# Li-Qingyun/RSCoTr

Hardware: AMD Instinct MI355X
Metric: images/sec MTL train step (Swin-T 512^2, bs=2/GPU) (higher is better)
Workload: dtype f32 (large products as three fp16 MFMAs on two-plane power-of-two-scaled splits of the fp32 operands, fp32 accumulate: fp32-FMA-class error; six bf16 MFMAs on three-plane splits where an operand has no range word)

## Files before the change

rscotr_amd/build.py:

```python
import hashlib
import os
import shutil
import subprocess
import sys

HERE = os.path.dirname(os.path.abspath(__file__))
CSRC = os.path.join(HERE, "csrc")
LIB = os.path.join(HERE, "librscotr.so")
STAMP = os.path.join(HERE, "librscotr.so.stamp")
ARCH = "gfx950"
FLAGS = ["-O3", "-std=c++17", "-fPIC", "-munsafe-fp-atomics", "-fno-fast-math",
         "-Wno-unused-result"]
HOST_FLAGS = ["-ffp-contract=off"]


def _sources():
    return sorted(os.path.join(CSRC, f) for f in os.listdir(CSRC)
                  if f.endswith(".hip") or f.endswith(".cpp"))


def _digest():
    h = hashlib.sha256()
    for p in _sources() + sorted(os.path.join(CSRC, f) for f in os.listdir(CSRC) if f.endswith(".h")) + \
            [os.path.join(HERE, "..", "include", "rscotr.h")]:
        h.update(p.encode())
        with open(p, "rb") as fh:
            h.update(fh.read())
    h.update(" ".join(FLAGS + HOST_FLAGS).encode())
    return h.hexdigest()


def find_hipcc():
    for cand in (os.environ.get("HIPCC"), shutil.which("hipcc"), "/opt/rocm/bin/hipcc"):
        if cand and os.path.exists(cand):
            return cand
    return None


def build_library(force=False, verbose=True):
    dig = _digest()
    if not force and os.path.exists(LIB) and os.path.exists(STAMP):
        with open(STAMP) as fh:
            if fh.read().strip() == dig:
                return LIB
    hipcc = find_hipcc()
    if hipcc is None:
        raise RuntimeError("hipcc not found: cannot build librscotr.so")
    objs = []
    objdir = os.path.join(HERE, "_obj")
    os.makedirs(objdir, exist_ok=True)
    procs = []
    hdr = hashlib.sha256()
    for h in sorted(os.path.join(CSRC, f) for f in os.listdir(CSRC) if f.endswith(".h")) + \
            [os.path.join(HERE, "..", "include", "rscotr.h")]:
        with open(h, "rb") as fh:
            hdr.update(fh.read())
    for src in _sources():
        obj = os.path.join(objdir, os.path.basename(src) + ".o")
        objs.append(obj)
        extra = HOST_FLAGS if src.endswith(".cpp") else []
        with open(src, "rb") as fh:
            odig = hashlib.sha256(fh.read() + hdr.digest() + " ".join(FLAGS + extra).encode()).hexdigest()
        ostamp = obj + ".stamp"
        if not force and os.path.exists(obj) and os.path.exists(ostamp) and open(ostamp).read().strip() == odig:
            continue
        with open(ostamp, "w") as fh:
            fh.write(odig)
        cmd = [hipcc, f"--offload-arch={ARCH}", *FLAGS, *extra, "-x", "hip", "-c", src, "-o", obj,
               "-I", CSRC, "-I", os.path.join(HERE, "..", "include")]
        if verbose:
            print("[rscotr build]", " ".join(cmd), flush=True)
        procs.append((src, subprocess.Popen(cmd, stdout=subprocess.PIPE, stderr=subprocess.STDOUT)))
    for src, p in procs:
        out, _ = p.communicate()
        if p.returncode != 0:
            os.remove(os.path.join(objdir, os.path.basename(src) + ".o.stamp"))
            raise RuntimeError(f"hipcc failed on {src}:\n{out.decode()}")
    cmd = [hipcc, f"--offload-arch={ARCH}", "-shared", "-fPIC", *objs, "-ldl", "-o", LIB]
    if verbose:
        print("[rscotr build]", " ".join(cmd), flush=True)
    subprocess.check_call(cmd)
    with open(STAMP, "w") as fh:
        fh.write(dig)
    return LIB


if __name__ == "__main__":
    build_library(force="--force" in sys.argv)
    print(LIB)
```

rscotr_amd/csrc/common.h:

```cpp
#pragma once
#include <hip/hip_runtime.h>
#include <stdint.h>
#include <stdio.h>
#include <stdarg.h>

#define RSCOTR_OK 0
#define RSCOTR_E_SHAPE (-1)
#define RSCOTR_E_ALIGN (-2)
#define RSCOTR_E_ARCH (-3)
#define RSCOTR_E_LAUNCH (-4)
#define RSCOTR_E_ARG (-5)

namespace rscotr {

char* err_buf();

inline int fail(int code, const char* fmt, ...) {
  va_list ap;
  va_start(ap, fmt);
  vsnprintf(err_buf(), 512, fmt, ap);
  va_end(ap);
  return code;
}

inline int check_launch(const char* what) {
  hipError_t e = hipGetLastError();
  if (e != hipSuccess) return fail(RSCOTR_E_LAUNCH, "%s: %s", what, hipGetErrorString(e));
  return RSCOTR_OK;
}

inline bool aligned16(const void* p) { return (reinterpret_cast<uintptr_t>(p) & 15u) == 0; }

constexpr int kWave = 64;

enum { PROF_GEMM = 0, PROF_MSDA_FWD = 1, PROF_MSDA_BWD = 2, PROF_HBM = 3, PROF_MFMA = 4, PROF_KINDS = 5 };
struct ProfScope {
  int slot;
  hipStream_t stream;
  ProfScope(int kind, double work, hipStream_t s, const char* fmt, ...);
  ~ProfScope();
};

template <int G>
__device__ __forceinline__ float group_sum(float v) {
#pragma unroll
  for (int o = G / 2; o > 0; o >>= 1) v += __shfl_xor(v, o, 64);
  return v;
}

template <int G>
__device__ __forceinline__ float group_max(float v) {
#pragma unroll
  for (int o = G / 2; o > 0; o >>= 1) v = fmaxf(v, __shfl_xor(v, o, 64));
  return v;
}

__device__ __forceinline__ float wave_sum(float v) { return group_sum<64>(v); }
__device__ __forceinline__ float wave_max(float v) { return group_max<64>(v); }

constexpr int kAmaxPlanes = 32;
constexpr int kAmaxStride = 16384;
constexpr int kRangeExpLo = 80;

__device__ __forceinline__ int range_byte(unsigned bits) {
  return min(max((int)((bits >> 23) & 0xffu), kRangeExpLo), kRangeExpLo + 4 * kAmaxPlanes - 1) - kRangeExpLo;
}
__device__ __forceinline__ void range_mark(unsigned* slot, int i) {
  reinterpret_cast<unsigned char*>(slot + (long)(i >> 2) * kAmaxStride)[i & 3] = 1;
}

__device__ __forceinline__ unsigned amax_fold(unsigned v) {
  int c = v ? 4 * (int)(threadIdx.x & (kAmaxPlanes - 1)) + ((31 - __clz((int)v)) >> 3) + 1 : 0;
#pragma unroll
  for (int o = kAmaxPlanes / 2; o > 0; o >>= 1) c = max(c, __shfl_xor(c, o, 64));
  c = __builtin_amdgcn_readfirstlane(c);
  return c ? (unsigned)(kRangeExpLo + c - 1) << 23 : 0u;
}
__device__ __forceinline__ unsigned amax_read(const unsigned* word) {
  return amax_fold(word[(long)(threadIdx.x & (kAmaxPlanes - 1)) * kAmaxStride]);
}
__device__ __forceinline__ float amax_hi(unsigned folded) { return folded ? __uint_as_float(folded + (1u << 23)) : 0.f; }

__device__ __forceinline__ void amax_commit(unsigned* slot, float amx) {
  if (!slot) return;
#pragma unroll
  for (int o = 32; o > 0; o >>= 1) amx = fmaxf(amx, __shfl_xor(amx, o, 64));
  if ((threadIdx.x & 63) == 0) {
    const unsigned b = __float_as_uint(amx) & 0x7fffffffu;
    if (b) range_mark(slot, range_byte(b));
  }
}

__device__ __forceinline__ float2 msda_location(const float* __restrict__ r, float2 o, const float* __restrict__ norm, int l, int P,
                                                int refdim) {
  float2 out;
  if (refdim == 2) {
    out.x = r[0] + o.x / norm[2 * l];
    out.y = r[1] + o.y / norm[2 * l + 1];
  } else {
    out.x = r[0] + o.x / (float)P * r[2] * 0.5f;
    out.y = r[1] + o.y / (float)P * r[3] * 0.5f;
  }
  return out;
}

__device__ __forceinline__ float amax4(float a, const float4& v) {
  return fmaxf(fmaxf(a, fmaxf(fabsf(v.x), fabsf(v.y))), fmaxf(fabsf(v.z), fabsf(v.w)));
}

}
```

rscotr_amd/csrc/gemm_h3.hip:

```cpp
#include "gemm_split_body.h"
#include "gemm_plan.h"

namespace rscotr {
template <int BM, int BN, bool AKM, bool BKM, int PIPE, bool EDGE = false, int OCC = 1, bool BPL = false>
__global__ __launch_bounds__(256, OCC) void gemm_h3_kernel(GemmParams p) {
  __shared__ __attribute__((aligned(16))) unsigned lds[bf16x6_lds_words<BM, BN, AKM, BKM, PIPE, true>()];
  gemm_bf16x6_body<BM, BN, AKM, BKM, PIPE, false, EDGE, true, BPL>(p, blockIdx.x, gridDim.x, lds);
}
template <bool AKM, bool BKM, bool EDGE = false>
__global__ __launch_bounds__(256) __attribute__((amdgpu_waves_per_eu(2, 2))) void gemm_h3_128_kernel(GemmParams p) {
  __shared__ __attribute__((aligned(16))) unsigned lds[bf16x6_lds_words<128, 128, AKM, BKM, 0, true>()];
  gemm_bf16x6_body<128, 128, AKM, BKM, 0, false, EDGE, true>(p, blockIdx.x, gridDim.x, lds);
}

void launch_h3(const GemmParams& p, const GemmPlan& pl, hipStream_t s) {
  if (pl.b_from_planes) {
    gemm_h3_kernel<64, 64, false, false, 2, false, 4, true><<<dim3(pl.nwg), 256, 0, s>>>(p);
    return;
  }
  with_split_cfg(pl, [&](auto bm, auto pipe, auto edge) {
    with_layout(pl.a_kmajor, pl.b_kmajor, [&](auto ak, auto bk) {
      constexpr int BM = decltype(bm)::value, PIPE = decltype(pipe)::value;
      constexpr bool EDGE = decltype(edge)::value, AK = decltype(ak)::value, BK = decltype(bk)::value;
      if constexpr (BM == 128) {
        gemm_h3_128_kernel<AK, BK, EDGE><<<dim3(pl.nwg), 256, 0, s>>>(p);
      } else if (PIPE == 2 && !EDGE && !AK) {
        gemm_h3_kernel<64, 64, false, BK, 2, false, 4><<<dim3(pl.nwg), 256, 0, s>>>(p);
      } else {
        gemm_h3_kernel<BM, BM, AK, BK, PIPE, EDGE><<<dim3(pl.nwg), 256, 0, s>>>(p);
      }
    });
  });
}
}
```

rscotr_amd/csrc/gemm_split_body.h:

```cpp
#pragma once
#include "gemm_common.h"
#include <type_traits>

namespace rscotr {
typedef __bf16 bf16x2_t __attribute__((ext_vector_type(2)));
template <int NPL>
__device__ __forceinline__ void split_pair(float a, float b, unsigned (&out)[3]) {
  const f32x2_t x = {a, b};
  const bf16x2_t h = __builtin_convertvector(x, bf16x2_t);
  out[0] = __builtin_bit_cast(unsigned, h);
  const f32x2_t r1 = x - __builtin_convertvector(h, f32x2_t);
  const bf16x2_t m = __builtin_convertvector(r1, bf16x2_t);
  out[1] = __builtin_bit_cast(unsigned, m);
  if (NPL == 3) {
    const f32x2_t r2 = r1 - __builtin_convertvector(m, f32x2_t);
    out[2] = __builtin_bit_cast(unsigned, __builtin_convertvector(r2, bf16x2_t));
  } else {
    out[2] = 0u;
  }
}

__device__ __forceinline__ unsigned cvt_pk_bf16(float lo, float hi) {
  const f32x2_t x = {lo, hi};
  return __builtin_bit_cast(unsigned, __builtin_convertvector(x, bf16x2_t));
}

template <int NPL>
__device__ __forceinline__ void split_rows4(const float4& e, const float4& o, uint4 (&out)[3]) {
  f32x2_t e01 = {e.x, e.y}, e23 = {e.z, e.w}, o01 = {o.x, o.y}, o23 = {o.z, o.w};
#pragma unroll
  for (int pl = 0; pl < NPL; ++pl) {
    const unsigned h0 = cvt_pk_bf16(e01.x, o01.x), h1 = cvt_pk_bf16(e01.y, o01.y);
    const unsigned h2 = cvt_pk_bf16(e23.x, o23.x), h3 = cvt_pk_bf16(e23.y, o23.y);
    out[pl] = make_uint4(h0, h1, h2, h3);
    if (pl + 1 < NPL) {
      const f32x2_t fe01 = {__uint_as_float(h0 << 16), __uint_as_float(h1 << 16)};
      const f32x2_t fe23 = {__uint_as_float(h2 << 16), __uint_as_float(h3 << 16)};
      const f32x2_t fo01 = {__uint_as_float(h0 & 0xffff0000u), __uint_as_float(h1 & 0xffff0000u)};
      const f32x2_t fo23 = {__uint_as_float(h2 & 0xffff0000u), __uint_as_float(h3 & 0xffff0000u)};
      e01 -= fe01; e23 -= fe23; o01 -= fo01; o23 -= fo23;
    }
  }
}

__device__ __forceinline__ void split_rows4_h(const float4& e, const float4& o, const H3Scale& k, uint4 (&out)[3]) {
  unsigned a[3], b[3], c[3], d[3];
  split_pair_h(e.x, o.x, k, a);
  split_pair_h(e.y, o.y, k, b);
  split_pair_h(e.z, o.z, k, c);
  split_pair_h(e.w, o.w, k, d);
  out[0] = make_uint4(a[0], b[0], c[0], d[0]);
  out[1] = make_uint4(a[1], b[1], c[1], d[1]);
}

template <int R, bool KM, int NPL, int SBK = 16, bool H16 = false>
struct SplitOperand {
  static_assert(!H16 || NPL == 2, "the fp16 split has two planes");
  static constexpr int LDR = SBK * NPL + 8;
  static constexpr int KP = SBK / 2;
  static constexpr int Q = SBK / 4;
  static constexpr int WORDS = KM ? NPL * KP * R : R * LDR / 2;
  static constexpr int ITEMS = KM ? KP * R / 4 : R * Q;
  static constexpr int NV = (ITEMS + 255) / 256;
  float4 v[NV], w[NV];

  template <bool EDGE = false>
  __device__ __forceinline__ void load(const float* __restrict__ P, int ld, int row0, int k0, int tid, int rlast = 0, int klim = 0) {
#pragma unroll
    for (int i = 0; i < NV; ++i) {
      const int idx = tid + i * 256;
      if (ITEMS % 256 == 0 || idx < ITEMS) {
        if (!KM) {
          const int row = EDGE ? min(row0 + idx / Q, rlast) : row0 + idx / Q;
          const int kk = k0 + (idx % Q) * 4;
          v[i] = *reinterpret_cast<const float4*>(P + (long)row * ld + (EDGE ? min(kk, klim - 4) : kk));
          if (EDGE && kk >= klim) v[i] = make_float4(0.f, 0.f, 0.f, 0.f);
        } else {
          const int kp = idx / (R / 4), r4 = (idx % (R / 4)) * 4;
          const int ka = k0 + 2 * kp, col = EDGE ? min(row0 + r4, rlast) : row0 + r4;
          if (!EDGE) {
            const float* src = P + (long)ka * ld + col;
            v[i] = *reinterpret_cast<const float4*>(src);
            w[i] = *reinterpret_cast<const float4*>(src + ld);
          } else {
            v[i] = *reinterpret_cast<const float4*>(P + (long)min(ka, klim - 1) * ld + col);
            w[i] = *reinterpret_cast<const float4*>(P + (long)min(ka + 1, klim - 1) * ld + col);
            if (ka >= klim) v[i] = make_float4(0.f, 0.f, 0.f, 0.f);
            if (ka + 1 >= klim) w[i] = make_float4(0.f, 0.f, 0.f, 0.f);
          }
        }
      }
    }
  }
  __device__ __forceinline__ void scale_k(const float* __restrict__ ks, int per, int k0, int tid, int klast = 0x7ffffffe) {
#pragma unroll
    for (int i = 0; i < NV; ++i) {
      const int idx = tid + i * 256;
      if (ITEMS % 256 == 0 || idx < ITEMS) {
        const int k = k0 + 2 * (idx / (R / 4));
        const float f0 = ks[min(k, klast) / per], f1 = ks[min(k + 1, klast) / per];
        v[i].x *= f0; v[i].y *= f0; v[i].z *= f0; v[i].w *= f0;
        w[i].x *= f1; w[i].y *= f1; w[i].z *= f1; w[i].w *= f1;
      }
    }
  }
  __device__ __forceinline__ void accum(float4& a, int tid, float f = 1.f) const {
    static_assert(!KM || 256 % (R / 4) == 0, "row sums assume one row group per thread");
#pragma unroll
    for (int i = 0; i < NV; ++i)
      if (ITEMS % 256 == 0 || tid + i * 256 < ITEMS) {
        a.x = fmaf(f, v[i].x + w[i].x, a.x); a.y = fmaf(f, v[i].y + w[i].y, a.y);
        a.z = fmaf(f, v[i].z + w[i].z, a.z); a.w = fmaf(f, v[i].w + w[i].w, a.w);
      }
  }
  __device__ __forceinline__ void store(unsigned* S, int tid, const H3Scale& hs = H3Scale{1.f, 2048.f}) const {
#pragma unroll
    for (int i = 0; i < NV; ++i) {
      const int idx = tid + i * 256;
      if (ITEMS % 256 == 0 || idx < ITEMS) {
        if (!KM) {
          const int row = idx / Q, kq = (idx % Q) * 4;
          unsigned ab[3], cd[3];
          if constexpr (H16) {
            split_pair_h(v[i].x, v[i].y, hs, ab);
            split_pair_h(v[i].z, v[i].w, hs, cd);
          } else {
            split_pair<NPL>(v[i].x, v[i].y, ab);
            split_pair<NPL>(v[i].z, v[i].w, cd);
          }
          unsigned* dst = S + (row * LDR + kq) / 2;
#pragma unroll
          for (int pl = 0; pl < NPL; ++pl) {
            uint2 q;
            q.x = ab[pl];
            q.y = cd[pl];
            *reinterpret_cast<uint2*>(dst + pl * (SBK / 2)) = q;
          }
        } else {
          const int kp = idx / (R / 4), r4 = (idx % (R / 4)) * 4;
          uint4 q[3];
          if constexpr (H16) split_rows4_h(v[i], w[i], hs, q);
          else split_rows4<NPL>(v[i], w[i], q);
#pragma unroll
          for (int pl = 0; pl < NPL; ++pl) *reinterpret_cast<uint4*>(S + (pl * KP + kp) * R + r4) = q[pl];
        }
      }
    }
  }
  static __device__ __forceinline__ void frag(const unsigned* S, int row, int g, int ks, bf16x8 (&f)[3]) {
    if (!KM) {
      const unsigned* q = S + (row * LDR + 16 * ks + 8 * g) / 2;
#pragma unroll
      for (int pl = 0; pl < NPL; ++pl) f[pl] = __builtin_bit_cast(bf16x8, *reinterpret_cast<const uint4*>(q + pl * (SBK / 2)));
    } else {
#pragma unroll
      for (int pl = 0; pl < NPL; ++pl) {
        const unsigned* q = S + (pl * KP + 8 * ks + 4 * g) * R + row;
        uint4 t;
        t.x = q[0]; t.y = q[R]; t.z = q[2 * R]; t.w = q[3 * R];
        f[pl] = __builtin_bit_cast(bf16x8, t);
      }
    }
  }
};

template <int R, int SBK>
struct PlaneOperandH {
  using Lay = SplitOperand<R, false, 2, SBK, true>;
  static_assert(R == 64 && SBK == 32, "one 32-byte piece per thread");
  static constexpr int WORDS = Lay::WORDS, KP = Lay::KP;
  typedef float vec4 __attribute__((ext_vector_type(4)));
  vec4 v0, v1;
  template <bool EDGE = false>
  __device__ __forceinline__ void load(const float* __restrict__ P, int ld, int row0, int k0, int tid, int = 0, int = 0) {
    const vec4* src = reinterpret_cast<const vec4*>(P) + ((long)(k0 / SBK) * ld + row0) * 8 + tid * 2;
    v0 = src[0];
    v1 = src[1];
  }
  __device__ __forceinline__ void store(unsigned* S, int tid, const H3Scale& = H3Scale{1.f, 2048.f}) const {
    vec4* dst = reinterpret_cast<vec4*>(S + (tid >> 2) * (Lay::LDR / 2) + (tid & 3) * 8);
    dst[0] = v0;
    dst[1] = v1;
  }
  static __device__ __forceinline__ void frag(const unsigned* S, int row, int g, int ks, bf16x8 (&f)[3]) { Lay::frag(S, row, g, ks, f); }
};

__device__ const float bf16x6_one = 1.f;
template <int PIPE> constexpr int bf16x6_bk() { return PIPE == 2 ? 32 : PIPE == 0 ? X6_BK0 : 16; }
constexpr int X6_D2 = 2, H3_VPM = 8, H3_DPM = 2;
template <int PIPE> constexpr int bf16x6_depth() { return PIPE == 2 ? X6_D2 : 1; }

template <int BM, int BN, bool AKM, bool BKM, int PIPE, bool H16 = false>
constexpr int bf16x6_lds_words() {
  constexpr int NPL = H16 ? 2 : 3;
  return (PIPE ? 2 : 1) * (SplitOperand<BM, AKM, NPL, bf16x6_bk<PIPE>(), H16>::WORDS + SplitOperand<BN, BKM, NPL, bf16x6_bk<PIPE>(), H16>::WORDS);
}

template <int BM, int BN, bool AKM, bool BKM, int PIPE, bool SLAB, bool EDGE = false, bool H16 = false, bool BPL = false>
__device__ __forceinline__ void gemm_bf16x6_body(GemmParams& p, const int bx, const int gx, unsigned* lds) {
  constexpr int NPL = H16 ? 2 : 3, SBK = bf16x6_bk<PIPE>(), D = bf16x6_depth<PIPE>();
  constexpr int MT = BM / 64, NT = BN / 64;
  using OA = SplitOperand<BM, AKM, NPL, SBK, H16>;
  static_assert(!BPL || (H16 && !BKM && !EDGE && PIPE == 2), "B from planes: the interior pipelined fp16 kernel");
  using OB = typename std::conditional<BPL, PlaneOperandH<BN, SBK>, SplitOperand<BN, BKM, NPL, SBK, H16>>::type;
  H3Scale ha{1.f, 2048.f}, hb{1.f, 2048.f};
  float inva = 1.f, invb = 1.f;
  unsigned ra = 0u, rb = 0u;
  if constexpr (H16) {
    ra = p.amax_a[(long)(threadIdx.x & (kAmaxPlanes - 1)) * kAmaxStride];
    rb = p.amax_b[(long)(threadIdx.x & (kAmaxPlanes - 1)) * kAmaxStride];
  }
  auto h3_scales = [&]() {
    if constexpr (H16) {
      const int ea = h3_scale_exp(amax_fold(ra)), eb = h3_scale_exp(amax_fold(rb));
      ha.sc = __uint_as_float((unsigned)ea << 23); ha.sc2 = __uint_as_float((unsigned)(ea + 11) << 23);
      hb.sc = __uint_as_float((unsigned)eb << 23); hb.sc2 = __uint_as_float((unsigned)(eb + 11) << 23);
      inva = __uint_as_float((unsigned)(254 - ea) << 23); invb = __uint_as_float((unsigned)(254 - eb) << 23);
    }
  };
  constexpr int NBUF = PIPE ? 2 : 1;
  unsigned* sA[2] = {lds, lds + (NBUF - 1) * OA::WORDS};
  unsigned* sB[2] = {lds + NBUF * OA::WORDS, lds + NBUF * OA::WORDS + (NBUF - 1) * OB::WORDS};
  const int tid = threadIdx.x, lane = tid & 63, wave = tid >> 6;
  const int wm = wave >> 1, wn = wave & 1;
  const int tiles_n = EDGE ? (p.N + BN - 1) / BN : p.N / BN;
  const int alast = EDGE ? (AKM ? p.M - 4 : p.M - 1) : 0, blast = EDGE ? (BKM ? p.N - 4 : p.N - 1) : 0;
  int tile, split = 0;
  if (p.splits == 1) {
    tile = xcd_swizzle(bx, gx);
  } else {
    const int x = bx & 7, j = bx >> 3;
    const int q = p.tiles >> 3, r = p.tiles & 7, run = q + (r ? 1 : 0);
    const int nt = q + (x < r ? 1 : 0);
    split = j / run;
    const int tl = j - split * run;
    if (tl >= nt) return;
    tile = (x < r ? x * (q + 1) : r * (q + 1) + (x - r) * q) + tl;
  }
  const int m0 = (tile / tiles_n) * BM, n0 = (tile % tiles_n) * BN;
  const int kbeg = split * p.ksplit_len;
  const int kend = min(p.K, kbeg + p.ksplit_len);
  const int nk = EDGE ? (kend - kbeg + SBK - 1) / SBK : (kend - kbeg) / SBK;
  const int klast = EDGE ? p.K - 1 : 0x7ffffffe;

  f32x16 acc[MT][NT];
  f32x16 acc2[H16 ? MT : 1][H16 ? NT : 1];
#pragma unroll
  for (int i = 0; i < MT; ++i)
#pragma unroll
    for (int j = 0; j < NT; ++j)
#pragma unroll
      for (int r = 0; r < 16; ++r) {
        acc[i][j][r] = 0.f;
        if constexpr (H16) acc2[i][j][r] = 0.f;
      }
  OA las[D];
  OB lbs[D];
  OA& la = las[0];
  OB& lb = lbs[0];
  const bool do_rs = AKM && p.rowsum && n0 == 0;
  float4 rs = make_float4(0.f, 0.f, 0.f, 0.f);
  const int fr = lane & 31, g = lane >> 5;
  auto fetch = [&](int t) {
    la.template load<EDGE>(p.A, p.lda, m0, kbeg + t * SBK, tid, alast, p.K);
    lb.template load<EDGE>(p.B, p.ldb, n0, kbeg + t * SBK, tid, blast, p.K);
    if (AKM && p.kscale) la.scale_k(p.kscale, p.krows_per, kbeg + t * SBK, tid, klast);
  };
  auto stage = [&](unsigned* a_s, unsigned* b_s) {
    if (AKM && do_rs) la.accum(rs, tid);
    la.store(a_s, tid, ha);
    lb.store(b_s, tid, hb);
  };
  auto mma = [&](const unsigned* a_s, const unsigned* b_s) {
#pragma unroll
    for (int ks = 0; ks < SBK / 16; ++ks) {
      bf16x8 af[MT][3], bf[NT][3];
#pragma unroll
      for (int i = 0; i < MT; ++i) OA::frag(a_s, wm * (BM / 2) + i * 32 + fr, g, ks, af[i]);
#pragma unroll
      for (int j = 0; j < NT; ++j) OB::frag(b_s, wn * (BN / 2) + j * 32 + fr, g, ks, bf[j]);
      if constexpr (H16) {
#pragma unroll
        for (int tm = 0; tm < 3; ++tm)
#pragma unroll
          for (int i = 0; i < MT; ++i)
#pragma unroll
            for (int j = 0; j < NT; ++j) {
              const f16x8 a = __builtin_bit_cast(f16x8, af[i][tm == 0 ? 1 : 0]), b = __builtin_bit_cast(f16x8, bf[j][tm == 1 ? 1 : 0]);
              if (tm < 2) acc2[i][j] = __builtin_amdgcn_mfma_f32_32x32x16_f16(a, b, acc2[i][j], 0, 0, 0);
              else acc[i][j] = __builtin_amdgcn_mfma_f32_32x32x16_f16(a, b, acc[i][j], 0, 0, 0);
            }
        continue;
      }
      constexpr int PA[6] = {2, 0, 1, 1, 0, 0}, PB[6] = {0, 2, 1, 0, 1, 0};
#pragma unroll
      for (int tm = 0; tm < 6; ++tm)
#pragma unroll
        for (int i = 0; i < MT; ++i)
#pragma unroll
          for (int j = 0; j < NT; ++j)
            acc[i][j] = __builtin_amdgcn_mfma_f32_32x32x16_bf16(af[i][PA[tm]], bf[j][PB[tm]], acc[i][j], 0, 0, 0);
    }
  };
  if (PIPE == 2) {
    constexpr int U = (D % 2 == 0) ? D : 2 * D;
    constexpr int NMFMA = MT * NT * (H16 ? 3 : 6) * (SBK / 16);
    constexpr int VPM = H16 ? H3_VPM : 4, DPM = H16 ? H3_DPM : 1;
    const float* ksp = (AKM && p.kscale) ? p.kscale : &bf16x6_one;
    const int ksper = (AKM && p.kscale) ? p.krows_per : 0x7fffffff;
#pragma unroll
    for (int d = 0; d < D; ++d) {
      const int tt = min(d, nk - 1);
      las[d].template load<EDGE>(p.A, p.lda, m0, kbeg + tt * SBK, tid, alast, p.K);
      lbs[d].template load<EDGE>(p.B, p.ldb, n0, kbeg + tt * SBK, tid, blast, p.K);
    }
    h3_scales();
    if (AKM) las[0].scale_k(ksp, ksper, kbeg, tid, klast);
    if (AKM) las[0].accum(rs, tid);
    las[0].store(sA[0], tid, ha);
    lbs[0].store(sB[0], tid, hb);
    __syncthreads();
    for (int t0 = 0; t0 < nk; t0 += U) {
#pragma unroll
      for (int s = 0; s < U; ++s) {
        const int t = t0 + s;
        if (t < nk) {
          {
            const int tt = min(t + D, nk - 1);
            las[s % D].template load<EDGE>(p.A, p.lda, m0, kbeg + tt * SBK, tid, alast, p.K);
            lbs[s % D].template load<EDGE>(p.B, p.ldb, n0, kbeg + tt * SBK, tid, blast, p.K);
          }
          mma(sA[s & 1], sB[s & 1]);
          if (AKM) las[(s + 1) % D].scale_k(ksp, ksper, kbeg + min(t + 1, nk - 1) * SBK, tid, klast);
          if (AKM) las[(s + 1) % D].accum(rs, tid, t + 1 < nk ? 1.f : 0.f);
          las[(s + 1) % D].store(sA[(s + 1) & 1], tid, ha);
          lbs[(s + 1) % D].store(sB[(s + 1) & 1], tid, hb);
#pragma unroll
          for (int i = 0; i < NMFMA; ++i) {
            __builtin_amdgcn_sched_group_barrier(0x008, 1, 0);
            __builtin_amdgcn_sched_group_barrier(0x002, VPM, 0);
            __builtin_amdgcn_sched_group_barrier(0x200, DPM, 0);
          }
          __syncthreads();
        }
      }
    }
  } else if (PIPE) {
    fetch(0);
    h3_scales();
    stage(sA[0], sB[0]);
    if (nk > 1) fetch(1);
    __syncthreads();
    for (int t = 0; t < nk; ++t) {
      const bool odd = t & 1;
      mma(odd ? sA[1] : sA[0], odd ? sB[1] : sB[0]);
      if (t + 1 < nk) {
        stage(odd ? sA[0] : sA[1], odd ? sB[0] : sB[1]);
        if (t + 2 < nk) fetch(t + 2);
      }
      __syncthreads();
    }
  } else {
    fetch(0);
    h3_scales();
    for (int t = 0; t < nk; ++t) {
      __syncthreads();
      stage(sA[0], sB[0]);
      if (t + 1 < nk) fetch(t + 1);
      __syncthreads();
      mma(sA[0], sB[0]);
    }
  }

  if (AKM && do_rs) {
    __syncthreads();
    constexpr int KL = 256 / (BM / 4) < OA::KP ? 256 / (BM / 4) : OA::KP;
    float4* red = reinterpret_cast<float4*>(lds);
    if (tid < KL * BM / 4) red[tid] = rs;
    __syncthreads();
    if (tid < BM) {
      const float* rf = reinterpret_cast<const float*>(lds);
      float v = 0.f;
#pragma unroll
      for (int k = 0; k < KL; ++k) v += rf[k * BM + tid];
      const int m = m0 + tid;
      if (!EDGE || m < p.M) {
        if (p.splits > 1 || SLAB) p.rs_slabs[(long)split * p.M + m] = v;
        else p.rowsum[m] = p.rowsum_acc ? p.rowsum[m] + v : v;
      }
    }
  }

  if constexpr (H16) {
#pragma unroll
    for (int i = 0; i < MT; ++i)
#pragma unroll
      for (int j = 0; j < NT; ++j)
#pragma unroll
        for (int r = 0; r < 16; ++r) acc[i][j][r] = fmaf(acc2[i][j][r], 0x1p-11f, acc[i][j][r]) * inva * invb;
  }
  if (p.splits > 1 || SLAB) {
    float* slab = p.slabs + (long)split * p.M * p.N;
#pragma unroll
    for (int i = 0; i < MT; ++i)
#pragma unroll
      for (int j = 0; j < NT; ++j) {
        const int n = n0 + wn * (BN / 2) + j * 32 + fr;
#pragma unroll
        for (int r = 0; r < 16; ++r) {
          const int m = m0 + wm * (BM / 2) + i * 32 + (r & 3) + 8 * (r >> 2) + 4 * g;
          if (!EDGE || (m < p.M && n < p.N)) slab[(long)m * p.N + n] = acc[i][j][r];
        }
      }
    return;
  }
  if constexpr (BM == 128 && BN == 128 && !EDGE) {
    if (p.act == ACT_RELU_BITS || p.act == ACT_RELU_GRAD_BITS) {
      const bool fwd = p.act == ACT_RELU_BITS;
      const long widx = ((long)(m0 / 128) * (p.N / 128) + n0 / 128) * 256 + tid;
      unsigned long long bits = fwd ? 0ull : reinterpret_cast<const unsigned long long*>(p.aux)[widx];
      float amx = 0.f;
#pragma unroll
      for (int i = 0; i < MT; ++i)
#pragma unroll
        for (int j = 0; j < NT; ++j) {
          const int n = n0 + wn * (BN / 2) + j * 32 + fr;
          const float bv = p.bias ? p.bias[n] : 0.f;
          float* crow = p.C + (long)(m0 + wm * (BM / 2) + i * 32 + 4 * g) * p.ldc + n;
#pragma unroll
          for (int r = 0; r < 16; ++r) {
            const int b = (i * NT + j) * 16 + r;
            float v = acc[i][j][r] + bv;
            if (fwd) {
              v = fmaxf(v, 0.f);
              bits |= (unsigned long long)(v > 0.f) << b;
            } else {
              v = ((bits >> b) & 1ull) ? v : 0.f;
            }
            crow[(long)((r & 3) + 8 * (r >> 2)) * p.ldc] = v;
            amx = fmaxf(amx, fabsf(v));
          }
        }
      if (fwd) reinterpret_cast<unsigned long long*>(p.pre)[widx] = bits;
      amax_commit(p.amax_out, amx);
      return;
    }
  }
  const bool plain = !p.pre && p.act == ACT_NONE && !p.resid && !p.accumulate && !p.rowscale && !p.C2;
  const bool one_extra = BM == 64 && !p.C2 &&
                         ((p.act == ACT_RELU_GRAD || p.act == ACT_GELU_GRAD) ? 1 : 0) + (p.resid ? 1 : 0) + (p.accumulate ? 1 : 0) == 1;
  const bool noload = !plain && (p.act == ACT_NONE || p.act == ACT_RELU || p.act == ACT_GELU) && !p.resid && !p.accumulate &&
                      !p.rowscale && !p.C2;
  float amx = 0.f;
#pragma unroll
  for (int i = 0; i < MT; ++i)
#pragma unroll
    for (int j = 0; j < NT; ++j) {
      const int n = n0 + wn * (BN / 2) + j * 32 + fr;
      if (EDGE && n >= p.N) continue;
      const float bv = p.bias ? p.bias[n] : 0.f;
      const int mb = m0 + wm * (BM / 2) + i * 32 + 4 * g;
      float* crow = p.C + (long)mb * p.ldc + n;
      if (one_extra) {
        epilogue_tile16<EDGE>(p, acc[i][j], bv, mb, n, amx);
        __builtin_amdgcn_sched_barrier(0);
      } else if (noload) {
        epilogue_noload16<EDGE>(p, acc[i][j], bv, mb, n, amx);
      } else if (plain) {
#pragma unroll
        for (int r = 0; r < 16; ++r)
          if (!EDGE || mb + (r & 3) + 8 * (r >> 2) < p.M) {
            const float v = acc[i][j][r] + bv;
            crow[(long)((r & 3) + 8 * (r >> 2)) * p.ldc] = v;
            amx = fmaxf(amx, fabsf(v));
          }
      } else {
#pragma unroll
        for (int g4 = 0; g4 < 4; ++g4) {
          float v[4];
#pragma unroll
          for (int u = 0; u < 4; ++u) v[u] = acc[i][j][4 * g4 + u] + bv;
          epilogue_rows4<EDGE>(p, v, mb + 8 * g4, n, amx);
          __builtin_amdgcn_sched_barrier(0);
        }
      }
    }
  amax_commit(p.amax_out, amx);
}
}
```

rscotr_amd/ops/deferred.py:

```python
import ctypes
from typing import NamedTuple

import numpy as np
import torch

from .._lib import _TRACE
from .core import ACT_NONE, _ptr, _stream, lib
from .ranges import RANGES
from .state import STATE


class Slab(NamedTuple):
    slab: int
    rs_slab: int
    out: int
    rowsum: int
    M: int
    N: int
    ldc: int
    splits: int


class LnPart(NamedTuple):
    part: int
    dw: int
    db: int
    rows: int
    C: int


class WattnPart(NamedTuple):
    part: int
    dtable: int
    dbias: int
    heads: int
    C: int
    rows: int


class GroupProblem(NamedTuple):
    a: int
    b: int
    out: int
    rowsum: int
    kscale: int
    M: int
    N: int
    K: int
    lda: int
    ldb: int
    krows_per: int
    range_a: int = 0
    range_b: int = 0


class _DeferredCombine:

    BLOCK = 256 << 20
    MAX_TABLES = 64
    GROUP_MAX_OUT = 160000
    GROUP_MAX_OUT_SHORT = 2500000
    GROUP_SHORT_K = 4096
    GROUP_EDGE = 48
    GROUP_TARGET_WGS = 4608

    def __init__(self):
        self.enabled = True
        self.blocks, self.cur, self.off = [], 0, 0
        self.entries, self.notify, self.cache = [], [], {}
        self.ln_entries, self.ln_cache = [], {}
        self.pin = False
        self.pinned = set()
        self.group_enabled = True
        self.group_x6 = 1
        self.group, self.group_keep, self.group_cache = [], [], {}
        self.group_amax, self.amax_cache = {}, {}
        self.pinned_pool, self.pinned_live = [], []
        self.captured = []
        self.wattn_entries, self.wattn_cache = [], {}

    def grouped_size(self, M, N, K):
        return M * N <= self.GROUP_MAX_OUT or (K <= self.GROUP_SHORT_K and M * N <= self.GROUP_MAX_OUT_SHORT)

    def split_member(self, M, N, K):
        return bool(self.group_x6 and K >= 512 and K % 16 == 0 and M % 4 == 0 and N % 4 == 0 and min(M, N) >= self.GROUP_EDGE)

    def _plan_group(self):
        probs = [GroupProblem(*p) for p in self.group]

        def kind(p):
            if not (self.split_member(p.M, p.N, p.K) and p.lda % 4 == 0 and p.ldb % 4 == 0 and p.a % 16 == 0 and p.b % 16 == 0):
                return 0
            return 7 if p.range_a and p.range_b and RANGES.enabled else 6

        def row(m, first):
            if m is None:
                return [0] * 12 + [first, 0, 0, 0]
            p = m['p']
            return [p.a, p.b, m['slab'], m['rs_slab'], p.kscale, p.M, p.N, p.K, p.lda, p.ldb, m['klen'], m['splits'], first,
                    max(p.krows_per, 1), m['ranges'], m['wgs']]

        kinds = [kind(p) for p in probs]
        tiles = [((p.M + 127) // 128) * ((p.N + 127) // 128) if k else ((p.M + 63) // 64) * ((p.N + 63) // 64)
                 for k, p in zip(kinds, probs)]
        dev = self.group_keep[0].device
        launches, ents = [], []
        for variant in (0, 6, 7):
            big = 4 if variant else 1
            klen_t = max(256, -(-sum(t * p.K * big for t, k, p in zip(tiles, kinds, probs) if k == variant) // self.GROUP_TARGET_WGS))
            kq = 32 if variant else 16
            members = []
            for t, k, p in zip(tiles, kinds, probs):
                if k != variant:
                    continue
                sp = max(1, -(-p.K // max(256, klen_t // big)))
                klen = -(-(-(-p.K // sp)) // kq) * kq
                sp = -(-p.K // klen)
                if sp == 1:
                    klen = p.K
                slab = self.reserve(sp * (p.M * p.N + p.M) * 4, dev)
                rs_slab = slab + sp * p.M * p.N * 4 if p.rowsum else 0
                rng = ((RANGES.index(p.range_a) + 1) << 32 | (RANGES.index(p.range_b) + 1)) if variant == 7 else 0
                members.append(dict(p=p, slab=slab, rs_slab=rs_slab, klen=klen, splits=sp, ranges=rng, wgs=t * sp))
                ents.append(Slab(slab, rs_slab, p.out, p.rowsum, p.M, p.N, p.N, sp))
            if members:
                members.sort(key=lambda m: -m['wgs'])
                members += [None] * (-len(members) % 8)
                rows, first = [], 0
                for b0 in range(0, len(members), 8):
                    rows += [row(m, first) for m in members[b0:b0 + 8]]
                    first += 8 * members[b0]['wgs']
                flops = float(sum(2.0 * m['p'].M * m['p'].N * m['p'].K for m in members if m is not None))
                launches.append((self._upload(np.asarray(rows, dtype=np.int64), dev), len(rows), first, variant, flops))
        return launches, ents

    def prepare_capture(self, n=4):
        while len(self.pinned_pool) < n:
            self.pinned_pool.append(torch.empty((4096, 16), dtype=torch.int64).pin_memory())

    @staticmethod
    def _copy(arr, dev):
        return torch.from_numpy(arr).to(dev)

    def _upload(self, arr, dev):
        if dev.type == 'cuda' and torch.cuda.is_current_stream_capturing():
            assert arr.size <= 4096 * 16, f'a table of {arr.size} words does not fit a staging buffer'
            assert self.pinned_pool, ('no staging buffer left for a table built during a capture: the pool is exhausted '
                                      f'({len(self.pinned_live)} taken), or DEFER.prepare_capture() did not run')
            host = self.pinned_pool.pop()
            stage = host.view(-1)[:arr.size].view(arr.shape)
            stage.copy_(torch.from_numpy(arr))
            d = torch.empty(arr.shape, dtype=torch.int64, device=dev)
            d.copy_(stage, non_blocking=True)
            self.pinned_live.append(host)
            return d
        return self._copy(arr, dev)

    def forget_captured(self):
        for cache, sig in self.captured:
            cache.pop(sig, None)
            self.pinned.discard(sig)
        self.captured = []

    def keep_captured(self):
        self.captured = []

    def _remember(self, cache, sig, hit):
        if sig not in cache and torch.cuda.is_available() and torch.cuda.is_current_stream_capturing():
            self.captured.append((cache, sig))
        if self.pin:
            self.pinned.add(sig)
        if sig not in cache:
            cache[sig] = hit
            if len(cache) > self.MAX_TABLES:
                for k in list(cache):
                    if len(cache) <= self.MAX_TABLES:
                        break
                    if k not in self.pinned and k != sig:
                        del cache[k]

    def reserve(self, nbytes, device):
        nbytes = (nbytes + 255) // 256 * 256
        while True:
            if self.cur == len(self.blocks):
                self.blocks.append(torch.empty(max(self.BLOCK, nbytes) // 4, dtype=torch.float32, device=device))
            b = self.blocks[self.cur]
            if self.off + nbytes <= b.numel() * 4:
                ptr = b.data_ptr() + self.off
                self.off += nbytes
                return ptr
            self.cur, self.off = self.cur + 1, 0

    def pending(self):
        return bool(self.entries or self.ln_entries or self.group or self.wattn_entries)

    def drop(self):
        self.entries, self.notify, self.ln_entries = [], [], []
        self.group, self.group_keep = [], []
        self.group_amax = {}
        self.wattn_entries = []
        self.cur = self.off = 0

    @staticmethod
    def _rounds(entries, dests):
        seen, rounds = {}, []
        for e in entries:
            ds = [d for d in dests(e) if d]
            k = max([seen.get(d, 0) for d in ds] or [0])
            for d in ds:
                seen[d] = k + 1
            while len(rounds) <= k:
                rounds.append([])
            rounds[k].append(e)
        return rounds

    def _flush_queue(self, entries, cache, kind, dests, plan, entry_point, upload):
        sig = tuple(entries)
        hit = cache.get(sig)
        if hit is None:
            dev = self.blocks[0].device
            hit = []
            for ents in self._rounds([kind(*e) for e in entries], dests):
                arrays, scalars = plan(ents)
                hit.append((tuple(upload(a, dev) for a in arrays), scalars))
        self._remember(cache, sig, hit)
        for tabs, scalars in hit:
            lib.call(entry_point, *(t.data_ptr() for t in tabs), *scalars, _stream())

    @staticmethod
    def _workgroups(ents, count):
        return np.asarray([(r, c) for r, e in enumerate(ents) for c in range(count(e))], dtype=np.int32)

    def _plan_ln(self, ents):
        wg = self._workgroups(ents, lambda e: (2 * e.C + 63) // 64)
        return (np.asarray(ents, dtype=np.int64), wg), (len(wg),)

    def _plan_wattn(self, ents):
        rows, first = [], 0
        for e in ents:
            rows.append(tuple(e) + (first,) + (0,) * 9)
            first += e.heads
        return (np.asarray(rows, dtype=np.int64),), (len(rows), first)

    def _plan_splitk(self, ents):
        wg = self._workgroups(ents, lambda e: (max(e.M * e.N // 4, e.M) + 255) // 256)
        nbytes = float(sum((e.splits + 2) * (e.M * e.N + e.M) * 4 for e in ents))
        return (np.asarray(ents, dtype=np.int64), wg), (len(wg), nbytes)

    def group_range(self, t, rows, cols, ld):
        s = RANGES.slot_of(t)
        if s:
            return s
        sink = STATE.grad_sink
        if sink is not None and sink.is_param_ptr(t.data_ptr()):
            return RANGES.of(t, rows, cols, ld)
        key = (t.data_ptr(), rows, cols, ld)
        s = self.group_amax.get(key)
        if s is None:
            s = self.group_amax[key] = RANGES.new_slot(t.device)
            if _TRACE:
                import sys
                end = t.storage_offset() * 4 + ((rows - 1) * ld + cols) * 4
                print(f'[group_range] {tuple(t.shape)} rows={rows} cols={cols} ld={ld} last byte {end} of storage {t.untyped_storage().nbytes()}'
                      + ('  <-- OUT OF BOUNDS' if end > t.untyped_storage().nbytes() else ''), file=sys.stderr, flush=True)
        return s

    def _measure_group(self):
        sig = tuple(self.group_amax.items())
        hit = self.amax_cache.get(sig)
        if hit is None:
            rows_, first = [], 0
            for (ptr, rows, cols, ld), slot in self.group_amax.items():
                rows_.append((ptr, rows, cols, ld, slot, first))
                first += max(1, min(128, rows * cols // 65536))
            hit = (self._upload(np.asarray(rows_, dtype=np.int64), self.group_keep[0].device), len(rows_), first)
        self._remember(self.amax_cache, sig, hit)
        table, n, total = hit
        lib.call('rscotr_amax_group', table.data_ptr(), n, total, _stream())
        RANGES.stats['grouped'] = RANGES.stats.get('grouped', 0) + n
        self.group_amax = {}

    def _flush_group(self):
        if self.group_amax:
            self._measure_group()
        sig = (tuple(self.group), self.cur, self.off)
        hit = self.group_cache.get(sig)
        if hit is None:
            hit = self._plan_group() + (self.cur, self.off)
        launches, ents, self.cur, self.off = hit
        self._remember(self.group_cache, sig, hit)
        for table, n, total, variant, flops in launches:
            lib.call('rscotr_gemm_dw_group', table.data_ptr(), n, total, variant, flops, RANGES.base if variant == 7 else 0,
                     _stream())
        self.entries.extend(ents)
        self.group, self.group_keep = [], []

    def flush(self):
        if self.group:
            self._flush_group()
        if self.ln_entries:
            self._flush_queue(self.ln_entries, self.ln_cache, LnPart, lambda e: (e.dw, e.db), self._plan_ln,
                              'rscotr_layernorm_flush', self._copy)
            self.ln_entries = []
        if self.wattn_entries:
            self._flush_queue(self.wattn_entries, self.wattn_cache, WattnPart, lambda e: (e.dtable, e.dbias), self._plan_wattn,
                              'rscotr_swin_wattn_flush', self._upload)
            self.wattn_entries = []
        if self.entries:
            self._flush_queue(self.entries, self.cache, Slab, lambda e: (e.out, e.rowsum), self._plan_splitk,
                              'rscotr_splitk_flush', self._copy)
        notify, self.notify = self.notify, []
        self.entries = []
        self.cur = self.off = 0
        if STATE.grad_sink is not None:
            for i in notify:
                STATE.grad_sink._on_ready(i)


DEFER = _DeferredCombine()


def _ranges_invalidated():
    DEFER.group = [GroupProblem(*p)._replace(range_a=0, range_b=0) for p in DEFER.group]
    DEFER.group_amax = {}


RANGES.on_invalidate.append(_ranges_invalidated)


def flush_deferred():
    if DEFER.pending() or DEFER.notify:
        DEFER.flush()


def _in_arena(t):
    sink = STATE.grad_sink
    if sink is None or t is None:
        return False
    lo = sink.flat_g.data_ptr()
    return lo <= t.data_ptr() < lo + sink.flat_g.numel() * 4


def _try_defer_dw(A, B, out, M, N, K, lda, ldb, rowsum, kscale, krows_per, nws):
    if not DEFER.enabled or STATE.side is not None or N % 4 or out.data_ptr() % 16 or not _in_arena(out):
        return False
    if DEFER.group_enabled and DEFER.grouped_size(M, N, K) and K >= 16:
        sa = sb = 0
        if DEFER.split_member(M, N, K) and RANGES.enabled:
            sa, sb = DEFER.group_range(A, K, M, lda), DEFER.group_range(B, K, N, ldb)
            lo_r, hi_r = RANGES.base, RANGES.base + 4 * RANGES.STRIDE
            if not (lo_r <= sa < hi_r and lo_r <= sb < hi_r):
                sa = sb = 0
        DEFER.group.append(GroupProblem(A.data_ptr(), B.data_ptr(), out.data_ptr(), _ptr(rowsum), _ptr(kscale), M, N, K, lda, ldb,
                                        int(krows_per), sa, sb))
        DEFER.group_keep.extend(t for t in (A, B, kscale) if t is not None)
        return True
    if nws == 0:
        return False
    ptr = DEFER.reserve(nws, A.device)
    splits = ctypes.c_int32(1)
    sa = sb = 0
    if RANGES.wanted(M, N, K, lda, ldb, 1, 1, ACT_NONE, False, False, kscale is not None, nws):
        sa, sb = RANGES.of(A, K, M, lda), RANGES.of(B, K, N, ldb)
    lib.call('rscotr_gemm_f32_dw_slabs_r', A.data_ptr(), B.data_ptr(), out.data_ptr(), M, N, K, lda, ldb, N, _ptr(rowsum),
             _ptr(kscale), int(krows_per), ptr, nws, ctypes.byref(splits), sa, sb, _stream())
    sp = splits.value
    if sp > 1:
        DEFER.entries.append(Slab(ptr, ptr + sp * M * N * 4 if rowsum is not None else 0, out.data_ptr(), _ptr(rowsum), M, N, N, sp))
    return True
```

Before: 210.6.

## Double-buffer register fetch sets in 128x128 fp16 split GEMM with buffer loads

For the 128x128 K-major fp16 three-MFMA GEMM kernel, the main loop now keeps two register sets of global loads in flight. The next tile's loads are issued while the current one is staged and multiplied. Loads use raw buffer loads with precomputed per-thread offsets and hardware bounds clamping, and k-scale factors are fetched ahead through the constant address space. Opaque asm barriers pin registers so the compiler does not spill. The build now checks resource-usage remarks and fails if these kernels use scratch. A fallback single-set variant handles leading dimensions of 2^26 or more, which overflow the 32-bit offsets, and the grouped planner avoids the range kind in that case. The cost is higher register pressure, at two waves per EU.

```diff
diff --git a/rscotr_amd/build.py b/rscotr_amd/build.py
--- a/rscotr_amd/build.py
+++ b/rscotr_amd/build.py
@@ -12,6 +12,18 @@
 FLAGS = ["-O3", "-std=c++17", "-fPIC", "-munsafe-fp-atomics", "-fno-fast-math",
          "-Wno-unused-result"]
 HOST_FLAGS = ["-ffp-contract=off"]
+REMARK_FLAGS = ["-Rpass-analysis=kernel-resource-usage"]
+NO_SCRATCH = {"gemm_h3.hip": ("gemm_h3_128_kernel",), "gemm_group.hip": ("gemm_h3_group_kernel",)}
+
+
+def scratch_report(remarks, names):
+    out, cur = {}, None
+    for line in remarks.splitlines():
+        if "Function Name:" in line:
+            cur = line.split("Function Name:")[1].split()[0]
+        elif "ScratchSize [bytes/lane]:" in line and cur is not None and any(n in cur for n in names):
+            out[cur] = int(line.split("ScratchSize [bytes/lane]:")[1].split()[0])
+    return out
 
 
 def _sources():
@@ -58,7 +70,7 @@
     for src in _sources():
         obj = os.path.join(objdir, os.path.basename(src) + ".o")
         objs.append(obj)
-        extra = HOST_FLAGS if src.endswith(".cpp") else []
+        extra = HOST_FLAGS if src.endswith(".cpp") else REMARK_FLAGS if os.path.basename(src) in NO_SCRATCH else []
         with open(src, "rb") as fh:
             odig = hashlib.sha256(fh.read() + hdr.digest() + " ".join(FLAGS + extra).encode()).hexdigest()
         ostamp = obj + ".stamp"
@@ -76,6 +88,14 @@
         if p.returncode != 0:
             os.remove(os.path.join(objdir, os.path.basename(src) + ".o.stamp"))
             raise RuntimeError(f"hipcc failed on {src}:\n{out.decode()}")
+        names = NO_SCRATCH.get(os.path.basename(src))
+        if names:
+            report = scratch_report(out.decode(), names)
+            spilled = {k: v for k, v in report.items() if v}
+            if not report or spilled:
+                os.remove(os.path.join(objdir, os.path.basename(src) + ".o.stamp"))
+                raise RuntimeError(f"{src}: kernels that must not use scratch do (bytes per lane: {spilled}), or no resource-usage "
+                                   f"remark was found for {names}: see h3_two_tiles in csrc/gemm_split_body.h")
     cmd = [hipcc, f"--offload-arch={ARCH}", "-shared", "-fPIC", *objs, "-ldl", "-o", LIB]
     if verbose:
         print("[rscotr build]", " ".join(cmd), flush=True)
diff --git a/rscotr_amd/csrc/common.h b/rscotr_amd/csrc/common.h
--- a/rscotr_amd/csrc/common.h
+++ b/rscotr_amd/csrc/common.h
@@ -69,12 +69,19 @@
   reinterpret_cast<unsigned char*>(slot + (long)(i >> 2) * kAmaxStride)[i & 3] = 1;
 }
 
+__device__ __forceinline__ int amax_fold_code(unsigned v, int sub) { return v ? 4 * sub + ((31 - __clz((int)v)) >> 3) + 1 : 0; }
+__device__ __forceinline__ unsigned amax_fold_bits(int c) { return c ? (unsigned)(kRangeExpLo + c - 1) << 23 : 0u; }
 __device__ __forceinline__ unsigned amax_fold(unsigned v) {
-  int c = v ? 4 * (int)(threadIdx.x & (kAmaxPlanes - 1)) + ((31 - __clz((int)v)) >> 3) + 1 : 0;
+  int c = amax_fold_code(v, (int)(threadIdx.x & (kAmaxPlanes - 1)));
 #pragma unroll
   for (int o = kAmaxPlanes / 2; o > 0; o >>= 1) c = max(c, __shfl_xor(c, o, 64));
-  c = __builtin_amdgcn_readfirstlane(c);
-  return c ? (unsigned)(kRangeExpLo + c - 1) << 23 : 0u;
+  return amax_fold_bits(__builtin_amdgcn_readfirstlane(c));
+}
+__device__ __forceinline__ unsigned amax_fold_lane(unsigned v, int lane) {
+  int c = amax_fold_code(v, lane & (kAmaxPlanes - 1));
+#pragma unroll
+  for (int o = kAmaxPlanes / 2; o > 0; o >>= 1) c = max(c, __builtin_amdgcn_ds_bpermute((lane ^ o) << 2, c));
+  return amax_fold_bits(__builtin_amdgcn_readfirstlane(c));
 }
 __device__ __forceinline__ unsigned amax_read(const unsigned* word) {
   return amax_fold(word[(long)(threadIdx.x & (kAmaxPlanes - 1)) * kAmaxStride]);
diff --git a/rscotr_amd/csrc/gemm_h3.hip b/rscotr_amd/csrc/gemm_h3.hip
--- a/rscotr_amd/csrc/gemm_h3.hip
+++ b/rscotr_amd/csrc/gemm_h3.hip
@@ -7,10 +7,10 @@
   __shared__ __attribute__((aligned(16))) unsigned lds[bf16x6_lds_words<BM, BN, AKM, BKM, PIPE, true>()];
   gemm_bf16x6_body<BM, BN, AKM, BKM, PIPE, false, EDGE, true, BPL>(p, blockIdx.x, gridDim.x, lds);
 }
-template <bool AKM, bool BKM, bool EDGE = false>
+template <bool AKM, bool BKM, bool EDGE = false, bool ONESET = false>
 __global__ __launch_bounds__(256) __attribute__((amdgpu_waves_per_eu(2, 2))) void gemm_h3_128_kernel(GemmParams p) {
   __shared__ __attribute__((aligned(16))) unsigned lds[bf16x6_lds_words<128, 128, AKM, BKM, 0, true>()];
-  gemm_bf16x6_body<128, 128, AKM, BKM, 0, false, EDGE, true>(p, blockIdx.x, gridDim.x, lds);
+  gemm_bf16x6_body<128, 128, AKM, BKM, 0, false, EDGE, true, false, ONESET>(p, blockIdx.x, gridDim.x, lds);
 }
 
 void launch_h3(const GemmParams& p, const GemmPlan& pl, hipStream_t s) {
@@ -23,7 +23,8 @@
       constexpr int BM = decltype(bm)::value, PIPE = decltype(pipe)::value;
       constexpr bool EDGE = decltype(edge)::value, AK = decltype(ak)::value, BK = decltype(bk)::value;
       if constexpr (BM == 128) {
-        gemm_h3_128_kernel<AK, BK, EDGE><<<dim3(pl.nwg), 256, 0, s>>>(p);
+        if (AK && BK && (p.lda >= (1 << 26) || p.ldb >= (1 << 26))) gemm_h3_128_kernel<AK, BK, EDGE, AK && BK><<<dim3(pl.nwg), 256, 0, s>>>(p);
+        else gemm_h3_128_kernel<AK, BK, EDGE><<<dim3(pl.nwg), 256, 0, s>>>(p);
       } else if (PIPE == 2 && !EDGE && !AK) {
         gemm_h3_kernel<64, 64, false, BK, 2, false, 4><<<dim3(pl.nwg), 256, 0, s>>>(p);
       } else {
diff --git a/rscotr_amd/csrc/gemm_split_body.h b/rscotr_amd/csrc/gemm_split_body.h
--- a/rscotr_amd/csrc/gemm_split_body.h
+++ b/rscotr_amd/csrc/gemm_split_body.h
@@ -92,6 +92,27 @@
       }
     }
   }
+  __device__ __forceinline__ unsigned thread_offset(int ld, int row0, int tid, bool edge, int rlast) const {
+    static_assert(!KM || ITEMS % 256 == 0, "whole items per thread");
+    const int col = row0 + (tid % (R / 4)) * 4;
+    return 4u * (unsigned)(2 * (tid / (R / 4)) * ld + (edge ? min(col, rlast) : col));
+  }
+  static __device__ __forceinline__ float4 load_row(const float* P, int ld, int krow, int klim, unsigned off) {
+    typedef unsigned vec4u __attribute__((ext_vector_type(4)));
+    const long left = 4l * ld * max(klim - krow, 0);
+    const __amdgpu_buffer_rsrc_t d = __builtin_amdgcn_make_buffer_rsrc(const_cast<float*>(P + (long)krow * ld), 0,
+                                                                        (int)(unsigned)min(left, 0xffffffffl), 0x00020000);
+    const vec4u t = __builtin_amdgcn_raw_buffer_load_b128(d, (int)off, 0, 0);
+    return make_float4(__uint_as_float(t.x), __uint_as_float(t.y), __uint_as_float(t.z), __uint_as_float(t.w));
+  }
+  __device__ __forceinline__ void load_rows(const float* __restrict__ P, int ld, int k0, int klim, unsigned off) {
+#pragma unroll
+    for (int i = 0; i < NV; ++i) {
+      const int krow = k0 + i * (2 * 256 / (R / 4));
+      v[i] = load_row(P, ld, krow, klim, off);
+      w[i] = load_row(P, ld, krow + 1, klim, off);
+    }
+  }
   __device__ __forceinline__ void scale_k(const float* __restrict__ ks, int per, int k0, int tid, int klast = 0x7ffffffe) {
 #pragma unroll
     for (int i = 0; i < NV; ++i) {
@@ -102,6 +123,32 @@
         v[i].x *= f0; v[i].y *= f0; v[i].z *= f0; v[i].w *= f0;
         w[i].x *= f1; w[i].y *= f1; w[i].z *= f1; w[i].w *= f1;
       }
+    }
+  }
+  __device__ __forceinline__ void scale_k_fetch(const float* __restrict__ ks, int per, int k0, int wave, int klast, float (&f)[4 * NV]) const {
+    static_assert(!KM || R == 128, "two k pairs per wavefront");
+#pragma unroll
+    for (int i = 0; i < NV; ++i) {
+      const int kb = k0 + 4 * wave + i * (2 * 256 / (R / 4));
+      int k = min(kb, klast), q = k / per, r = k - q * per;
+#pragma unroll
+      for (int j = 0; j < 4; ++j) {
+        const int kn = min(kb + j, klast);
+        if (kn != k) {
+          k = kn;
+          if (++r == per) { r = 0; ++q; }
+        }
+        f[4 * i + j] = *(const __attribute__((address_space(4))) float*)(ks + q);
+      }
+    }
+  }
+  __device__ __forceinline__ void scale_k_apply(const float (&f)[4 * NV], int tid) {
+    const bool hi = (tid / (R / 4)) & 1;
+#pragma unroll
+    for (int i = 0; i < NV; ++i) {
+      const float f0 = hi ? f[4 * i + 2] : f[4 * i], f1 = hi ? f[4 * i + 3] : f[4 * i + 1];
+      v[i].x *= f0; v[i].y *= f0; v[i].z *= f0; v[i].w *= f0;
+      w[i].x *= f1; w[i].y *= f1; w[i].z *= f1; w[i].w *= f1;
     }
   }
   __device__ __forceinline__ void accum(float4& a, int tid, float f = 1.f) const {
@@ -189,6 +236,8 @@
 template <int PIPE> constexpr int bf16x6_bk() { return PIPE == 2 ? 32 : PIPE == 0 ? X6_BK0 : 16; }
 constexpr int X6_D2 = 2, H3_VPM = 8, H3_DPM = 2;
 template <int PIPE> constexpr int bf16x6_depth() { return PIPE == 2 ? X6_D2 : 1; }
+template <int BM, int BN, bool AKM, bool BKM, int PIPE, bool EDGE, bool H16>
+constexpr bool h3_two_tiles() { return H16 && PIPE == 0 && BM == 128 && BN == 128 && AKM && BKM; }
 
 template <int BM, int BN, bool AKM, bool BKM, int PIPE, bool H16 = false>
 constexpr int bf16x6_lds_words() {
@@ -196,9 +245,10 @@
   return (PIPE ? 2 : 1) * (SplitOperand<BM, AKM, NPL, bf16x6_bk<PIPE>(), H16>::WORDS + SplitOperand<BN, BKM, NPL, bf16x6_bk<PIPE>(), H16>::WORDS);
 }
 
-template <int BM, int BN, bool AKM, bool BKM, int PIPE, bool SLAB, bool EDGE = false, bool H16 = false, bool BPL = false>
+template <int BM, int BN, bool AKM, bool BKM, int PIPE, bool SLAB, bool EDGE = false, bool H16 = false, bool BPL = false, bool ONESET = false>
 __device__ __forceinline__ void gemm_bf16x6_body(GemmParams& p, const int bx, const int gx, unsigned* lds) {
-  constexpr int NPL = H16 ? 2 : 3, SBK = bf16x6_bk<PIPE>(), D = bf16x6_depth<PIPE>();
+  constexpr bool TWO = !ONESET && h3_two_tiles<BM, BN, AKM, BKM, PIPE, EDGE, H16>();
+  constexpr int NPL = H16 ? 2 : 3, SBK = bf16x6_bk<PIPE>(), D = TWO ? 2 : bf16x6_depth<PIPE>();
   constexpr int MT = BM / 64, NT = BN / 64;
   using OA = SplitOperand<BM, AKM, NPL, SBK, H16>;
   static_assert(!BPL || (H16 && !BKM && !EDGE && PIPE == 2), "B from planes: the interior pipelined fp16 kernel");
@@ -212,7 +262,14 @@
   }
   auto h3_scales = [&]() {
     if constexpr (H16) {
-      const int ea = h3_scale_exp(amax_fold(ra)), eb = h3_scale_exp(amax_fold(rb));
+      if constexpr (TWO) {
+        int ln = (int)__lane_id();
+        asm volatile("" : "+v"(ln));
+        ra = amax_fold_lane(ra, ln); rb = amax_fold_lane(rb, ln);
+      } else {
+        ra = amax_fold(ra); rb = amax_fold(rb);
+      }
+      const int ea = h3_scale_exp(ra), eb = h3_scale_exp(rb);
       ha.sc = __uint_as_float((unsigned)ea << 23); ha.sc2 = __uint_as_float((unsigned)(ea + 11) << 23);
       hb.sc = __uint_as_float((unsigned)eb << 23); hb.sc2 = __uint_as_float((unsigned)(eb + 11) << 23);
       inva = __uint_as_float((unsigned)(254 - ea) << 23); invb = __uint_as_float((unsigned)(254 - eb) << 23);
@@ -221,8 +278,8 @@
   constexpr int NBUF = PIPE ? 2 : 1;
   unsigned* sA[2] = {lds, lds + (NBUF - 1) * OA::WORDS};
   unsigned* sB[2] = {lds + NBUF * OA::WORDS, lds + NBUF * OA::WORDS + (NBUF - 1) * OB::WORDS};
-  const int tid = threadIdx.x, lane = tid & 63, wave = tid >> 6;
-  const int wm = wave >> 1, wn = wave & 1;
+  int tid = threadIdx.x, lane = tid & 63, wave = tid >> 6;
+  int wm = wave >> 1, wn = wave & 1;
   const int tiles_n = EDGE ? (p.N + BN - 1) / BN : p.N / BN;
   const int alast = EDGE ? (AKM ? p.M - 4 : p.M - 1) : 0, blast = EDGE ? (BKM ? p.N - 4 : p.N - 1) : 0;
   int tile, split = 0;
@@ -260,7 +317,7 @@
   OB& lb = lbs[0];
   const bool do_rs = AKM && p.rowsum && n0 == 0;
   float4 rs = make_float4(0.f, 0.f, 0.f, 0.f);
-  const int fr = lane & 31, g = lane >> 5;
+  int fr = lane & 31, g = lane >> 5;
   auto fetch = [&](int t) {
     la.template load<EDGE>(p.A, p.lda, m0, kbeg + t * SBK, tid, alast, p.K);
     lb.template load<EDGE>(p.B, p.ldb, n0, kbeg + t * SBK, tid, blast, p.K);
@@ -272,13 +329,15 @@
     lb.store(b_s, tid, hb);
   };
   auto mma = [&](const unsigned* a_s, const unsigned* b_s) {
+    int ra0 = wm * (BM / 2) + fr, rb0 = wn * (BN / 2) + fr;
+    if constexpr (TWO) asm volatile("" : "+v"(ra0), "+v"(rb0));
 #pragma unroll
     for (int ks = 0; ks < SBK / 16; ++ks) {
       bf16x8 af[MT][3], bf[NT][3];
 #pragma unroll
-      for (int i = 0; i < MT; ++i) OA::frag(a_s, wm * (BM / 2) + i * 32 + fr, g, ks, af[i]);
-#pragma unroll
-      for (int j = 0; j < NT; ++j) OB::frag(b_s, wn * (BN / 2) + j * 32 + fr, g, ks, bf[j]);
+      for (int i = 0; i < MT; ++i) OA::frag(a_s, ra0 + i * 32, g, ks, af[i]);
+#pragma unroll
+      for (int j = 0; j < NT; ++j) OB::frag(b_s, rb0 + j * 32, g, ks, bf[j]);
       if constexpr (H16) {
 #pragma unroll
         for (int tm = 0; tm < 3; ++tm)
@@ -360,6 +419,56 @@
       }
       __syncthreads();
     }
+  } else if constexpr (TWO) {
+    float kf[4 * OA::NV];
+    const unsigned offa = la.thread_offset(p.lda, m0, tid, EDGE, alast);
+    const unsigned offb = lb.thread_offset(p.ldb, n0, tid, EDGE, blast);
+    const int wave_u = __builtin_amdgcn_readfirstlane(tid >> 6);
+    auto factors = [&](int t) {
+      if (p.kscale) la.scale_k_fetch(p.kscale, p.krows_per, kbeg + t * SBK, wave_u, klast, kf);
+    };
+    auto fetch2 = [&](auto set, int t) {
+      constexpr int S = decltype(set)::value;
+      const int k0 = __builtin_amdgcn_readfirstlane(kbeg + t * SBK);
+      las[S].load_rows(p.A, p.lda, k0, kend, offa);
+      lbs[S].load_rows(p.B, p.ldb, k0, kend, offb);
+    };
+    auto stage2 = [&](auto set) {
+      constexpr int S = decltype(set)::value;
+#pragma unroll
+      for (int i = 0; i < OA::NV; ++i) {
+        asm volatile("" : "+v"(las[S].v[i].x), "+v"(las[S].v[i].y), "+v"(las[S].v[i].z), "+v"(las[S].v[i].w));
+        asm volatile("" : "+v"(las[S].w[i].x), "+v"(las[S].w[i].y), "+v"(las[S].w[i].z), "+v"(las[S].w[i].w));
+        asm volatile("" : "+v"(lbs[S].v[i].x), "+v"(lbs[S].v[i].y), "+v"(lbs[S].v[i].z), "+v"(lbs[S].v[i].w));
+        asm volatile("" : "+v"(lbs[S].w[i].x), "+v"(lbs[S].w[i].y), "+v"(lbs[S].w[i].z), "+v"(lbs[S].w[i].w));
+      }
+      if (p.kscale) las[S].scale_k_apply(kf, tid);
+      if (do_rs) las[S].accum(rs, tid);
+      las[S].store(sA[0], tid, ha);
+      lbs[S].store(sB[0], tid, hb);
+    };
+    constexpr std::integral_constant<int, 0> s0{};
+    constexpr std::integral_constant<int, 1> s1{};
+    factors(0);
+    fetch2(s0, 0);
+    fetch2(s1, 1);
+    h3_scales();
+    for (int t = 0; t < nk; t += 2) {
+      __syncthreads();
+      stage2(s0);
+      if (t + 1 < nk) factors(t + 1);
+      fetch2(s0, t + 2);
+      __syncthreads();
+      mma(sA[0], sB[0]);
+      if (t + 1 < nk) {
+        __syncthreads();
+        stage2(s1);
+        if (t + 2 < nk) factors(t + 2);
+        fetch2(s1, t + 3);
+        __syncthreads();
+        mma(sA[0], sB[0]);
+      }
+    }
   } else {
     fetch(0);
     h3_scales();
@@ -372,6 +481,10 @@
     }
   }
 
+  if constexpr (TWO) {
+    asm volatile("" : "+v"(tid));
+    lane = tid & 63; wave = tid >> 6; wm = wave >> 1; wn = wave & 1; fr = lane & 31; g = lane >> 5;
+  }
   if (AKM && do_rs) {
     __syncthreads();
     constexpr int KL = 256 / (BM / 4) < OA::KP ? 256 / (BM / 4) : OA::KP;
diff --git a/rscotr_amd/ops/deferred.py b/rscotr_amd/ops/deferred.py
--- a/rscotr_amd/ops/deferred.py
+++ b/rscotr_amd/ops/deferred.py
@@ -91,7 +91,7 @@
         def kind(p):
             if not (self.split_member(p.M, p.N, p.K) and p.lda % 4 == 0 and p.ldb % 4 == 0 and p.a % 16 == 0 and p.b % 16 == 0):
                 return 0
-            return 7 if p.range_a and p.range_b and RANGES.enabled else 6
+            return 7 if p.range_a and p.range_b and RANGES.enabled and max(p.lda, p.ldb) < 1 << 26 else 6
 
         def row(m, first):
             if m is None:
```

New measurement: 213.0 (median of 6 runs). 1.1% higher.
